# mcmilk/7-Zip-zstd

Measured on AMD Instinct MI355X. Metric: compress MB/s + ratio-vs-ref, enwik9 zstd-L3 & Silesia flzma2-L5 (value = the zstd-L3 enwik9 leg; flzma2_l5_silesia = the other leg), higher is better.
Workload: dtype u8; 1 GPU; zstd level 3, enwik9 stand-in (text-zipf, 1000000000 B), 128 KiB blocks in independent 8 MiB match-finder frames; bytes_total=1000000000

## Files before the change

7-zip-zstd_amd/csrc/gc_lz_window.hip:

```cpp
#include "gc_mf.h"
#include "gc_lz_parse.h"
#ifdef HIPEMU
#include <stdio.h>
#include <stdlib.h>
#endif

#ifdef GC_MF_FAST
#define MFK(name) name##_p8
#else
#define MFK(name) name
#endif

namespace MFK(gc_mf_ns) {

#define MF_T         GC_MF_PARTS
static_assert(MF_T == GC_MF_PARTS, "W1 uses one thread per partition for the histogram row");
#define MF_PWAVES    (GC_MF_PARTS / 64u)
#define MFS_T        GC_MF_SCATTER_T
#define MFS_WAVES    (MFS_T / 64u)
#define MFS_ROUNDS   (GC_MF_TILE / MFS_T)
static_assert(MFS_T >= GC_MF_PARTS && MFS_T % 64u == 0u && GC_MF_TILE % (2u * MFS_T) == 0u && GC_MF_PARTS < 0xFFFFu, "W3: the first GC_MF_PARTS threads do the offsets; whole rounds, two per register");
#define MF_STAGE_PAD 16u
#define MF_STAGE_WORDS ((GC_MF_TILE + 2u * MF_STAGE_PAD + 32u) / 4u)

// ... 226 lines not shown
    }
    __syncthreads();
    GcMfEntry* E = ent + (uint64_t)T.frame * ((uint64_t)MF_F(frameBlocks) * GC_ZSTD_BLOCK_MAX);
    for (uint32_t j = t; j < nEnt; j += MFS_T) {
        const MfKeys k = mf_keys<MODE>(sW, sPerm[j], T);
        E[sDelta[k.part] + j] = k.entry;
    }
}
extern "C" __global__ void __launch_bounds__(MFS_T)
MFK(gc_mf_scatter_kernel)(const uint8_t* __restrict__ src, uint64_t srcSize, uint32_t frameBlocks, uint32_t nTiles, uint32_t per,
                     const uint32_t* __restrict__ offs, GcMfEntry* __restrict__ ent)
{
    mf_scatter_body<MF_BASE>(src, srcSize, frameBlocks, nTiles, per, offs, ent);
}
extern "C" __global__ void __launch_bounds__(MFS_T)
MFK(gc_mf_scatter_short_kernel)(const uint8_t* __restrict__ src, uint64_t srcSize, uint32_t frameBlocks, uint32_t nTiles, uint32_t per,
                           const uint32_t* __restrict__ offs, GcMfEntry* __restrict__ ent)
{
    mf_scatter_body<MF_SHORT>(src, srcSize, frameBlocks, nTiles, per, offs, ent);
}
extern "C" __global__ void __launch_bounds__(MFS_T)
MFK(gc_mf_scatter_far_kernel)(const uint8_t* __restrict__ src, uint64_t srcSize, uint32_t frameBlocks, uint32_t nTiles, uint32_t per,
                         const uint32_t* __restrict__ offs, GcMfEntry* __restrict__ ent)
{
    mf_scatter_body<MF_FAR>(src, srcSize, frameBlocks, nTiles, per, offs, ent);
}
extern "C" __global__ void __launch_bounds__(MFS_T)
MFK(gc_mf_scatter_far2_kernel)(const uint8_t* __restrict__ src, uint64_t srcSize, uint32_t frameBlocks, uint32_t nTiles, uint32_t per,
                         const uint32_t* __restrict__ offs, GcMfEntry* __restrict__ ent)
{
    mf_scatter_body<MF_FAR2>(src, srcSize, frameBlocks, nTiles, per, offs, ent);
}

#ifndef LINK_DEPTH
#define LINK_DEPTH 8u
#endif
#ifdef GC_MF_FAST
#define LINK_SEG   49152u
#else
#define LINK_SEG   16384u
#endif
#define LINK_WARM  16384u
#define LINK_SEGS  GC_MF_LINK_SEGS
#define LINK_BATCH 16u

__device__ __forceinline__ uint32_t mf_link_pick(uint32_t seen, uint32_t mine)
{
    return (seen != 0u && seen < mine && ((seen ^ mine) & ((1u << GC_MF_TAG_BITS) - 1u)) == 0u) ? (seen >> GC_MF_TAG_BITS) : 0u;
}

__device__ __forceinline__ void mf_link_load(uint64_t q[LINK_DEPTH], const GcMfEntry* __restrict__ E, uint32_t s0, uint32_t end, uint32_t lane)
{
#pragma unroll
    for (uint32_t d = 0; d < LINK_DEPTH; d++) {
        const uint32_t i = s0 + d * 64u + lane;
        q[d] = E[i < end ? i : end - 1u];
    }
}

__device__ __forceinline__ void mf_link_steps(const uint64_t q[LINK_DEPTH], uint32_t* tabL, uint32_t* tabS, GcMfEntry* __restrict__ EO, uint32_t s0,
                                              uint32_t end, uint32_t lane)
{
    if (s0 >= end) return;
    uint32_t pos[LINK_DEPTH], mL[LINK_DEPTH], mS[LINK_DEPTH], rL[LINK_DEPTH], rS[LINK_DEPTH];
#pragma unroll
    for (uint32_t d = 0; d < LINK_DEPTH; d++) {
        const uint32_t i = s0 + d * 64u + lane;
        const uint64_t e = q[d];
        pos[d] = (uint32_t)e & ((1u << GC_MF_POS_BITS) - 1u);
        const uint32_t kL = (uint32_t)(e >> GC_MF_POS_BITS) & ((1u << GC_MF_KL_BITS) - 1u);
        const uint32_t kS = (uint32_t)(e >> (GC_MF_POS_BITS + GC_MF_KL_BITS)) & ((1u << GC_MF_KS_BITS) - 1u);
        mL[d] = ((pos[d] + 1u) << GC_MF_TAG_BITS) | (kL & ((1u << GC_MF_TAG_BITS) - 1u)); mS[d] = ((pos[d] + 1u) << GC_MF_TAG_BITS) | (kS & ((1u << GC_MF_TAG_BITS) - 1u));
        rL[d] = 0; rS[d] = 0;
        if (i < end) { rL[d] = atomicMax(&tabL[kL >> (GC_MF_KL_BITS - GC_MF_LSLOT_LOG)], mL[d]); rS[d] = atomicMax(&tabS[kS >> (GC_MF_KS_BITS - GC_MF_SSLOT_LOG)], mS[d]); }
        gc_wave_step();
    }
#pragma unroll
    for (uint32_t d = 0; d < LINK_DEPTH; d++) {
        const uint32_t i = s0 + d * 64u + lane;
        const uint32_t cL = mf_link_pick(rL[d], mL[d]), cS = mf_link_pick(rS[d], mS[d]);
        if (i < end) EO[i] = (uint64_t)(pos[d] & (GC_MF_TILE - 1u)) | ((uint64_t)cL << GC_MF_TILE_LOG) | ((uint64_t)cS << (GC_MF_TILE_LOG + GC_MF_CAND_BITS));
    }
}

extern "C" __global__ void __launch_bounds__(64)
MFK(gc_mf_link_kernel)(const uint32_t* __restrict__ offs, const GcMfEntry* __restrict__ ent, GcMfEntry* __restrict__ entOut, uint32_t tilesPerFrame,
                  uint64_t frameBytes, uint32_t nLists, uint32_t* __restrict__ ticket)
{
    __shared__ uint32_t tabL[1u << GC_MF_LSLOT_LOG];
    __shared__ uint32_t tabS[1u << GC_MF_SSLOT_LOG];
    const uint32_t lane = threadIdx.x;
    const uint32_t nUpper = nLists * (LINK_SEGS - 1u), nBatches = (nUpper + LINK_BATCH - 1u) / LINK_BATCH, nTickets = nBatches + nLists;
    for (;;) {
        uint32_t tk = 0;
        if (lane == 0u) tk = atomicAdd(ticket, 1u);
        tk = __shfl(tk, 0);
        if (tk >= nTickets) break;
        uint64_t todo;
        uint32_t myItem, myStart = 0, myEnd = 0;
        {
            myItem = tk < nBatches ? tk * LINK_BATCH + lane : nUpper + (tk - nBatches);
            const bool inRange = tk < nBatches ? (lane < LINK_BATCH && myItem < nUpper) : lane == 0u;
            bool exists = false;
            if (inRange) {
                const uint32_t seg = LINK_SEGS - 1u - myItem / nLists, fg = myItem % nLists;
                const uint32_t frame = fg >> GC_MF_PART_LOG, g = fg & (GC_MF_PARTS - 1u);
                const uint32_t* row = offs + (uint64_t)frame * (tilesPerFrame + 1u) * GC_MF_PARTS;
                const uint32_t listStart = row[g], listEnd = row[(uint64_t)tilesPerFrame * GC_MF_PARTS + g];
                myStart = listStart + seg * LINK_SEG;
                exists = myStart < listEnd;
                myEnd = (seg + 1u < LINK_SEGS && myStart + LINK_SEG < listEnd) ? myStart + LINK_SEG : listEnd;
            }
            todo = __ballot(exists);
        }
      while (todo != 0ull) {
        const uint32_t src_ = gc_ctz64(todo);
        todo &= todo - 1ull;
        const uint32_t item = __shfl(myItem, (int)src_), start = __shfl(myStart, (int)src_), end = __shfl(myEnd, (int)src_);
        const uint32_t seg = LINK_SEGS - 1u - item / nLists, fg = item % nLists;
        const uint32_t frame = fg >> GC_MF_PART_LOG;
        const GcMfEntry* E = ent + (uint64_t)frame * frameBytes;
        GcMfEntry* EO = entOut + (uint64_t)frame * frameBytes;
        gc_wave_sync();
        for (uint32_t i = lane; i < (1u << GC_MF_LSLOT_LOG); i += 64u) tabL[i] = 0;
        for (uint32_t i = lane; i < (1u << GC_MF_SSLOT_LOG); i += 64u) tabS[i] = 0;
        gc_wave_sync();
        if (seg != 0u) {
            for (uint32_t i = start - LINK_WARM + lane; i < start; i += 64u) {
                const uint64_t e = E[i];
                const uint32_t pos = (uint32_t)e & ((1u << GC_MF_POS_BITS) - 1u);
                const uint32_t kL = (uint32_t)(e >> GC_MF_POS_BITS) & ((1u << GC_MF_KL_BITS) - 1u);
                const uint32_t kS = (uint32_t)(e >> (GC_MF_POS_BITS + GC_MF_KL_BITS)) & ((1u << GC_MF_KS_BITS) - 1u);
                atomicMax(&tabL[kL >> (GC_MF_KL_BITS - GC_MF_LSLOT_LOG)], ((pos + 1u) << GC_MF_TAG_BITS) | (kL & ((1u << GC_MF_TAG_BITS) - 1u)));
                atomicMax(&tabS[kS >> (GC_MF_KS_BITS - GC_MF_SSLOT_LOG)], ((pos + 1u) << GC_MF_TAG_BITS) | (kS & ((1u << GC_MF_TAG_BITS) - 1u)));
            }
            gc_wave_sync();
        }
        uint64_t qa[LINK_DEPTH], qb[LINK_DEPTH];
        mf_link_load(qa, E, start, end, lane);
        for (uint32_t s0 = start; s0 < end; s0 += 2u * 64u * LINK_DEPTH) {
            mf_link_load(qb, E, s0 + 64u * LINK_DEPTH, end, lane);
            mf_link_steps(qa, tabL, tabS, EO, s0, end, lane);
            mf_link_load(qa, E, s0 + 2u * 64u * LINK_DEPTH, end, lane);
            mf_link_steps(qb, tabL, tabS, EO, s0 + 64u * LINK_DEPTH, end, lane);
        }
      }
    }
}

#define MFV_T GC_MF_VERIFY_T
#ifndef MFV_B
#define MFV_B 4u
#endif
#define MFV_NONE 0xFFFFFFFFu
#define MFV_PAD_AFTER (GC_MATCH_CAP + 32u)
#define MFV_STAGE_WORDS ((MF_STAGE_PAD + GC_MF_TILE + MFV_PAD_AFTER) / 4u)

__device__ __forceinline__ LzW16 mf_lds_ld16(const uint32_t* sW, uint32_t i)
{
    LzW16 w; w.a = mf_lds_ld64(sW, i); w.b = mf_lds_ld64(sW, i + 8u); return w;
}
__device__ __forceinline__ uint32_t mfv_len16(const LzW16& me, const LzW16& cw, uint32_t maxLen, uint32_t minLen = GC_MIN_MATCH)
{
    uint32_t len = lz_cmp16(me, cw);
    if (len > maxLen) len = maxLen;
    return len >= minLen ? len : 0u;
}

#define MFV_BACK 3u
__device__ __forceinline__ uint32_t mfv_len13(const LzW16& me, const LzW16& cw, uint32_t maxLen, uint32_t& ext, uint32_t minLen = GC_MIN_MATCH)
{
    const uint64_t d0 = me.a ^ cw.a, d1 = me.b ^ cw.b;
    const bool b2 = ((d0 >> 16) & 0xFFull) == 0ull, b1 = ((d0 >> 8) & 0xFFull) == 0ull, b0 = (d0 & 0xFFull) == 0ull;
    ext = b2 ? (b1 ? (b0 ? 3u : 2u) : 1u) : 0u;
    const uint64_t e0 = (d0 >> 24) | (d1 << 40), e1 = (d1 >> 24) | (1ull << 40);
    uint32_t len = e0 ? gc_ctz64(e0) >> 3 : 8u + (gc_ctz64(e1) >> 3);
    if (len > maxLen) len = maxLen;
    return len >= minLen ? len : 0u;
}

#define VP_PHASE(prof, tprev, i) do { if ((prof) != nullptr && threadIdx.x == 0) { const unsigned long long now_ = gc_clock(); atomicAdd(&(prof)[i], now_ - (tprev)); (tprev) = now_; } } while (0)

#define MFV_CATCH 3u
#define MFV_XBITS 0x80u
template <int MODE, bool TILE_LIMIT = false, bool BACK = false>
__device__ __forceinline__ void mf_verify_tile(const MfTile& T, const uint8_t* __restrict__ src, uint64_t srcSize, uint32_t frameBlocks,
                    const uint32_t* __restrict__ offs, const GcMfEntry* __restrict__ ent, const uint32_t* recIn,
                    uint32_t* sW, uint32_t* sRec, uint8_t* sExt, uint32_t* sStart, uint32_t* sLocal, uint32_t* sWaveTot,
                    unsigned long long* prof = nullptr, unsigned long long* tprev = nullptr,
                    const uint32_t* __restrict__ changedIn = nullptr )
{
    constexpr bool FAR = MODE == MF_FAR || MODE == MF_FAR2 || MODE == MF_SHORT;
    constexpr bool SHIFT = BACK;
    constexpr uint32_t MINLEN = MODE == MF_SHORT ? 3u : GC_MIN_MATCH;
    constexpr uint32_t LONGLEN = MODE == MF_SHORT ? 4u : ((MODE == MF_FAR || MODE == MF_FAR2) ? 16u : 8u);
    const uint32_t t = threadIdx.x, lane = t & 63u, wave = t >> 6;
    const uint32_t TPF = MF_F(frameBlocks) * GC_MF_TILES_PER_BLOCK;
    uint32_t c = 0, incl = 0;
    if (t < GC_MF_PARTS) {
        const uint32_t* row = offs + ((uint64_t)T.frame * (TPF + 1u) + T.tif) * GC_MF_PARTS;
        const uint32_t o = row[t];
        c = row[GC_MF_PARTS + t] - o;
        sStart[t] = o;
        incl = gc_wave_incl_sum(c);
        if (lane == 63u) sWaveTot[wave] = incl;
    }
    mf_stage(sW, MFV_STAGE_WORDS, src, srcSize, T.tileStart, t, MFV_T);
    uint32_t* const sDirty = (uint32_t*)sExt;
    uint32_t* const sBack2 = (uint32_t*)(sExt + GC_MF_TILE / 8u + 16u);
    if (BACK) { for (uint32_t i = t; i < GC_MF_TILE / 32u; i += MFV_T) sBack2[i] = 0u; }
    if (FAR) {
        const GcU4* R4 = (const GcU4*)(recIn + T.tileStart);
        GcU4* S4 = (GcU4*)sRec;
        for (uint32_t i = t; i < (T.len + 3u) / 4u; i += MFV_T) S4[i] = R4[i];
        const uint32_t* D = changedIn != nullptr ? changedIn + (T.tileStart >> 5) : (const uint32_t*)nullptr;
        const uint32_t nW = (T.len + 31u) / 32u;
        for (uint32_t i = t; i < GC_MF_TILE / 32u + 4u; i += MFV_T) sDirty[i] = D != nullptr ? ((i < nW ? D[i] : 0u) | ((i >= 2u && i - 2u < nW) ? D[i - 2u] : 0u)) : 0u;
    } else {
        GcU4 none; none.x = none.y = none.z = none.w = MFV_NONE;
        GcU4* S4 = (GcU4*)sRec;
        for (uint32_t i = t; i < GC_MF_TILE / 4u; i += MFV_T) S4[i] = none;
    }
    __syncthreads();
    if (t < GC_MF_PARTS) {
        uint32_t before = 0;
        for (uint32_t w = 0; w < GC_MF_PARTS / 64u; w++) if (w < wave) before += sWaveTot[w];
        sLocal[t] = before + incl - c;
        if (t == GC_MF_PARTS - 1u) sLocal[GC_MF_PARTS] = before + incl;
    }
    __syncthreads();
    const uint32_t nEnt = sLocal[GC_MF_PARTS];
    VP_PHASE(prof, *tprev, 0);
    const uint8_t* wsrc = src + T.frameStart;
    const GcMfEntry* E = ent + (uint64_t)T.frame * ((uint64_t)MF_F(frameBlocks) * GC_ZSTD_BLOCK_MAX);
    const uint64_t blockBase = T.tileStart & ~(uint64_t)(GC_ZSTD_BLOCK_MAX - 1u);
    const uint32_t nBlk = (uint32_t)((srcSize - blockBase) < GC_ZSTD_BLOCK_MAX ? (srcSize - blockBase) : GC_ZSTD_BLOCK_MAX);
    const uint32_t pTile = (uint32_t)(T.tileStart - blockBase);
    const uint32_t wTile = (uint32_t)(T.tileStart - T.frameStart);
    auto unlisted = [&]() {
        for (uint32_t q = t; q < T.len; q += MFV_T) {
            if (!FAR && sRec[q] != MFV_NONE) continue;
            const uint64_t x = mf_lds_ld64(sW, q + MF_STAGE_PAD);
            const bool run = T.tileStart + q > T.frameStart && ((x << 8) | (uint64_t)mf_lds_byte(sW, q + MF_STAGE_PAD - 1u)) == x;
            const bool windowed = T.tileStart + q + GC_MATCH_CAP + 16u <= T.frameEnd;
            if (windowed && !run) continue;
            const uint32_t p = pTile + q;
            uint32_t len = 0;
            if (run && windowed && p + 8u <= nBlk) {
                uint32_t maxLen = (nBlk - p) < GC_MATCH_CAP ? (nBlk - p) : GC_MATCH_CAP;
                if (TILE_LIMIT && maxLen > T.len - q) maxLen = T.len - q;
                while (len < maxLen) {
                    const uint32_t more = lz_cmp16(mf_lds_ld16(sW, q + MF_STAGE_PAD + len), mf_lds_ld16(sW, q + MF_STAGE_PAD - 1u + len));
                    len += more;
                    if (more < 16u) break;
                }
                if (len > maxLen) len = maxLen;
                if (len < GC_MIN_MATCH) len = 0;
            }
            sRec[q] = len ? ((1u << 8) | len) : 0u;
        }
    };
    const uint32_t stagedLo = wTile >= MF_STAGE_PAD ? wTile - MF_STAGE_PAD : wTile + 0xFFFFFFFFu , stagedHi = wTile + (MFV_STAGE_WORDS * 4u - MF_STAGE_PAD);
    auto ld16c = [&](uint64_t c) -> LzW16 {
        if (wTile >= MF_STAGE_PAD && c >= stagedLo && c + 20u <= stagedHi) return mf_lds_ld16(sW, (uint32_t)(c - stagedLo));
        return lz_ld16(wsrc, c);
    };
    const uint32_t perWave = ((nEnt + MFV_T - 1u) / MFV_T) * 64u;
    const uint32_t jBeg = wave * perWave, jEnd = jBeg + perWave < nEnt ? jBeg + perWave : nEnt;
    uint32_t g0 = 0;
    if (jBeg < jEnd) {
#pragma unroll
        for (uint32_t step = GC_MF_PARTS / 2u; step != 0u; step >>= 1) if (sLocal[g0 + step] <= jBeg) g0 += step;
    }
    for (uint32_t j0 = jBeg; j0 < jEnd; j0 += 64u * MFV_B) {
        uint64_t e[MFV_B];
        bool live[MFV_B];
#pragma unroll
        for (uint32_t k = 0; k < MFV_B; k++) {
            const uint32_t j = j0 + k * 64u + lane;
            live[k] = j < jEnd;
            const uint32_t jj = live[k] ? j : jEnd - 1u;
            uint32_t lo = g0;
            while (sLocal[lo + 1u] <= jj) lo++;
            e[k] = E[sStart[lo] + (jj - sLocal[lo])];
            g0 = gc_readlane(lo, 63u);
        }
        uint32_t q[MFV_B], cS[MFV_B], maxLen[MFV_B], bestLen[MFV_B], bestC[MFV_B];
        uint32_t bestExt[MFV_B];
        LzW16 cw[MFV_B];
#pragma unroll
        for (uint32_t k = 0; k < MFV_B; k++) {
            q[k] = (uint32_t)e[k] & (GC_MF_TILE - 1u);
            const uint32_t cL = (uint32_t)(e[k] >> GC_MF_TILE_LOG) & ((1u << GC_MF_CAND_BITS) - 1u);
            cS[k] = (uint32_t)(e[k] >> (GC_MF_TILE_LOG + GC_MF_CAND_BITS)) & ((1u << GC_MF_CAND_BITS) - 1u);
            const uint32_t p = pTile + q[k];
            const bool can = live[k] && p + 8u <= nBlk;
            maxLen[k] = can ? ((nBlk - p) < GC_MATCH_CAP ? (nBlk - p) : GC_MATCH_CAP) : 0u;
            if (TILE_LIMIT && maxLen[k] > T.len - q[k]) maxLen[k] = T.len - q[k];
            if (cS[k] == cL) cS[k] = 0;
            bestC[k] = (can && cL) ? cL : 0u;
            bestExt[k] = 0;
            if (SHIFT) { if (bestC[k] <= MFV_BACK) bestC[k] = 0; if (cS[k] <= MFV_BACK) cS[k] = 0; }
            if (bestC[k]) cw[k] = ld16c(bestC[k] - 1u - (SHIFT ? MFV_BACK : 0u));
        }
#pragma unroll
        for (uint32_t k = 0; k < MFV_B; k++) {
            if (SHIFT) { uint32_t x = 0; bestLen[k] = bestC[k] ? mfv_len13(mf_lds_ld16(sW, q[k] + MF_STAGE_PAD - MFV_BACK), cw[k], maxLen[k], x, MINLEN) : 0u; bestExt[k] = (BACK && x > q[k]) ? q[k] : x; }
            else bestLen[k] = bestC[k] ? mfv_len16(mf_lds_ld16(sW, q[k] + MF_STAGE_PAD), cw[k], maxLen[k], MINLEN) : 0u;
            if (bestLen[k] >= (SHIFT && LONGLEN > 13u ? 13u : LONGLEN) || maxLen[k] == 0u) cS[k] = 0;
            if (cS[k]) cw[k] = ld16c(cS[k] - 1u - (SHIFT ? MFV_BACK : 0u));
        }
#pragma unroll
        for (uint32_t k = 0; k < MFV_B; k++) {
            const uint32_t pw = wTile + q[k];
            if (cS[k]) {
                uint32_t x = 0;
                const uint32_t len = SHIFT ? mfv_len13(mf_lds_ld16(sW, q[k] + MF_STAGE_PAD - MFV_BACK), cw[k], maxLen[k], x, MINLEN) : mfv_len16(mf_lds_ld16(sW, q[k] + MF_STAGE_PAD), cw[k], maxLen[k], MINLEN);
                if (BACK && x > q[k]) x = q[k];
                if (len && (bestLen[k] == 0u || lz_gain(len, pw - (cS[k] - 1u)) > lz_gain(bestLen[k], pw - (bestC[k] - 1u)))) { bestLen[k] = len; bestC[k] = cS[k]; bestExt[k] = x; }
            }
            uint32_t len = bestLen[k];
            while ((SHIFT ? (len & 15u) == 13u : (len >= 16u && (len & 15u) == 0u)) && len < maxLen[k]) {
                const uint32_t more = lz_cmp16(mf_lds_ld16(sW, q[k] + MF_STAGE_PAD + len), ld16c((uint64_t)(bestC[k] - 1u) + len));
                len += more;
                if (len > maxLen[k]) len = maxLen[k];
                if (more < 16u) break;
            }
            if (live[k]) {
                const uint32_t nr = len ? (((pw - (bestC[k] - 1u)) << 8) | len) : 0u;
                if (MODE == MF_BASE && len == GC_MATCH_CAP) sWaveTot[1] = 0xFFFFFFFFu;
                const uint32_t xb = (BACK && nr != 0u) ? ((bestExt[k] & 1u) << 7) : 0u;
                const bool x2 = BACK && nr != 0u && (bestExt[k] & 2u) != 0u;
                if (!FAR) { sRec[q[k]] = nr | xb; if (x2) atomicOr(&sBack2[q[k] >> 5], 1u << (q[k] & 31u)); }
                else if (nr) {
                    const uint32_t old = sRec[q[k]];
                    bool take = old == 0u || lz_gain(len, nr >> 8) > lz_gain(old & 0xFFu, old >> 8);
                    if (MODE == MF_FAR2 && old != 0u && len == GC_MATCH_CAP && (old & 0xFFu) == GC_MATCH_CAP && (old >> 8) != (nr >> 8)) {
                        const uint64_t frameLen = T.frameEnd - T.frameStart;
                        const uint64_t room = frameLen - ((uint64_t)pw + GC_MATCH_CAP);
                        const uint32_t lim = room < 80u ? (room < 16u ? 0u : (uint32_t)room - 16u) : 64u;
                        uint32_t eN = 0, eO = 0;
                        const uint64_t own = (uint64_t)pw + GC_MATCH_CAP;
                        while (eN < lim) { const uint32_t m = lz_cmp16(lz_ld16(wsrc, own + eN), lz_ld16(wsrc, own - (nr >> 8) + eN)); eN += m; if (m < 16u) break; }
                        while (eO < lim) { const uint32_t m = lz_cmp16(lz_ld16(wsrc, own + eO), lz_ld16(wsrc, own - (old >> 8) + eO)); eO += m; if (m < 16u) break; }
                        if (eN > lim) eN = lim; if (eO > lim) eO = lim;
                        take = eN > eO || (eN == eO && (nr >> 8) < (old >> 8));
                    }
                    if (take) {
                        sRec[q[k]] = nr | xb; if (x2) atomicOr(&sBack2[q[k] >> 5], 1u << (q[k] & 31u));
                        atomicOr(&sDirty[q[k] >> 5], 1u << (q[k] & 31u)); atomicOr(&sDirty[(q[k] + GC_MATCH_CAP) >> 5], 1u << ((q[k] + GC_MATCH_CAP) & 31u));
                    }
                }
            }
        }
    }
    VP_PHASE(prof, *tprev, 1);
    if (!FAR) { __syncthreads(); unlisted(); }
    if (BACK) {
        __syncthreads();
        constexpr uint32_t NSUBC = MFV_T / 64u;
        const uint32_t shareLen = GC_MF_TILE / NSUBC, cBeg = wave * shareLen, cEnd = cBeg + shareLen;
        uint32_t beyond[MFV_CATCH];
#pragma unroll
        for (uint32_t j = 0; j < MFV_CATCH; j++) beyond[j] = cEnd + j < T.len ? sRec[cEnd + j] : 0u;
        __syncthreads();
        for (uint32_t x0 = cBeg; x0 < cEnd && x0 < T.len; x0 += 64u) {
            const uint32_t x = x0 + lane;
            const uint32_t old = x < T.len ? sRec[x] : 0u;
            const uint32_t own = old & ~MFV_XBITS;
            uint32_t best = own;
            int bg = (own & 0xFFu) ? lz_gain(own & 0xFFu, own >> 8) : -100000;
#pragma unroll
            for (uint32_t j = 1; j <= MFV_CATCH; j++) {
                const uint32_t y = x + j;
                uint32_t ry = (y < cEnd && y < T.len) ? sRec[y] : 0u;
                if (y >= cEnd) ry = y - cEnd == 0u ? beyond[0] : (y - cEnd == 1u ? beyond[1] : beyond[2]);
                const uint32_t e = (ry & 0x7Fu) == 0u ? 0u : (((ry >> 7) & 1u) | (((sBack2[(y & (GC_MF_TILE - 1u)) >> 5] >> (y & 31u)) & 1u) << 1));
                if (e >= j) {
                    uint32_t l = (ry & 0x7Fu) + j; if (l > GC_MATCH_CAP) l = GC_MATCH_CAP;
                    const uint32_t off = ry >> 8;
                    const int g = lz_gain(l, off);
                    if (g > bg) { bg = g; best = (off << 8) | l; }
                }
            }
            gc_wave_sync();
            if (x < T.len && old != best) {
                sRec[x] = best;
                if (own != best) {
                    if (FAR) { atomicOr(&sDirty[x >> 5], 1u << (x & 31u)); atomicOr(&sDirty[(x + GC_MATCH_CAP) >> 5], 1u << ((x + GC_MATCH_CAP) & 31u)); }
                    if (MODE == MF_BASE && (best & 0xFFu) == GC_MATCH_CAP) sWaveTot[1] = 0xFFFFFFFFu;
                }
            }
            gc_wave_sync();
        }
    }
    __syncthreads();
    if ((MODE == MF_BASE && sWaveTot[1] == 0xFFFFFFFFu) || MODE == MF_FAR || MODE == MF_FAR2 || MODE == MF_SHORT) {
        constexpr uint32_t NSUB = MFV_T / 64u;
        const uint32_t subLen = ((T.len + NSUB * 64u - 1u) / (NSUB * 64u)) * 64u;
        const uint32_t sBeg = wave * subLen, sEnd = sBeg + subLen < T.len ? sBeg + subLen : T.len;
        auto piece4 = [&](uint32_t q, uint64_t cpos, uint32_t maxLen, const LzW16& c0, const LzW16& c1, const LzW16& c2, const LzW16& c3) -> uint32_t {
            const bool h1 = 16u < maxLen, h2 = 32u < maxLen, h3 = 48u < maxLen;
            uint32_t more = lz_cmp16(mf_lds_ld16(sW, q + MF_STAGE_PAD), c0);
            bool full = more == 16u;
            if (full && h1) { const uint32_t m = lz_cmp16(mf_lds_ld16(sW, q + MF_STAGE_PAD + 16u), c1); more += m; full = m == 16u; }
            if (full && h2) { const uint32_t m = lz_cmp16(mf_lds_ld16(sW, q + MF_STAGE_PAD + 32u), c2); more += m; full = m == 16u; }
            if (full && h3) { const uint32_t m = lz_cmp16(mf_lds_ld16(sW, q + MF_STAGE_PAD + 48u), c3); more += m; full = m == 16u; }
            (void)cpos;
            return more > maxLen ? maxLen : more;
        };
        auto walk = [&](uint32_t q, const uint32_t qEnd, const bool follow) {
            while (q < qEnd) {
                const uint32_t prev = sRec[q - GC_MATCH_CAP];
                const uint32_t d = prev >> 8, cur = sRec[q];
                const uint32_t p = pTile + q;
                const bool fresh = !FAR || ((sDirty[q >> 5] >> (q & 31u)) & 1u) != 0u;
                const bool need0 = fresh && (prev & 0xFFu) == GC_MATCH_CAP && (cur >> 8) != d && d <= wTile + q
                                   && T.tileStart + q + GC_MATCH_CAP + 16u <= T.frameEnd && p + 8u <= nBlk;
                if (!need0) { if (follow) return; q += 64u; continue; }
                uint32_t max0 = (nBlk - p) < GC_MATCH_CAP ? (nBlk - p) : GC_MATCH_CAP;
                if (TILE_LIMIT && max0 > T.len - q) max0 = T.len - q;
                const uint64_t cpos = (uint64_t)(wTile + q) - d;
                const uint32_t q1 = q + 64u;
                uint32_t cur1 = 0u;
                bool spec = max0 == GC_MATCH_CAP && q1 < qEnd;
                if (spec) {
                    cur1 = sRec[q1];
                    spec = (cur1 >> 8) != d && T.tileStart + q1 + GC_MATCH_CAP + 16u <= T.frameEnd && p + 64u + GC_MATCH_CAP <= nBlk && (!TILE_LIMIT || q1 + GC_MATCH_CAP <= T.len);
                }
                const bool h1 = 16u < max0, h2 = 32u < max0, h3 = 48u < max0;
                const LzW16 c0 = lz_ld16(wsrc, cpos), c1 = lz_ld16(wsrc, cpos + (h1 ? 16u : 0u)), c2 = lz_ld16(wsrc, cpos + (h2 ? 32u : 0u)), c3 = lz_ld16(wsrc, cpos + (h3 ? 48u : 0u));
                LzW16 e0 = c0, e1 = c0, e2 = c0, e3 = c0;
                if (spec) { e0 = lz_ld16(wsrc, cpos + 64u); e1 = lz_ld16(wsrc, cpos + 80u); e2 = lz_ld16(wsrc, cpos + 96u); e3 = lz_ld16(wsrc, cpos + 112u); }
                const uint32_t len0 = piece4(q, cpos, max0, c0, c1, c2, c3);
                if (len0 < MINLEN || len0 + 2u < (cur & 0xFFu)) { if (follow) return; q += 64u; continue; }
                sRec[q] = (d << 8) | len0;
                if (FAR) atomicOr(&sDirty[q1 >> 5], 1u << (q1 & 31u));
                if (!(spec && len0 == GC_MATCH_CAP)) { q += 64u; continue; }
                const uint32_t len1 = piece4(q1, cpos + 64u, GC_MATCH_CAP, e0, e1, e2, e3);
                if (len1 < MINLEN || len1 + 2u < (cur1 & 0xFFu)) { if (follow) return; q += 128u; continue; }
                sRec[q1] = (d << 8) | len1;
                if (FAR) atomicOr(&sDirty[(q1 + 64u) >> 5], 1u << ((q1 + 64u) & 31u));
                q += 128u;
            }
        };
        walk(sBeg + GC_MATCH_CAP + lane, sEnd, false);
        __syncthreads();
        const uint32_t qFirst = sBeg + lane;
        const uint32_t prevA = (wave != 0u && qFirst < sEnd) ? sRec[qFirst - GC_MATCH_CAP] : 0u;
        __syncthreads();
        if (wave != 0u) walk(qFirst, sEnd, true);
        __syncthreads();
        for (uint32_t sIdx = 2; sIdx < NSUB; sIdx++) {
            if (wave == sIdx && qFirst < sEnd && sRec[qFirst - GC_MATCH_CAP] != prevA) walk(qFirst, sEnd, true);
            __syncthreads();
        }
    }
}

template <int MODE, bool BACK = true>
__device__ __forceinline__ void mf_verify_body(const uint8_t* __restrict__ src, uint64_t srcSize, uint32_t frameBlocks, uint32_t nTiles, uint32_t per,
                    const uint32_t* __restrict__ offs, const GcMfEntry* __restrict__ ent, const uint32_t* recIn, uint32_t* rec, const uint32_t* __restrict__ changedIn = nullptr)
{
    __shared__ uint32_t sW[MFV_STAGE_WORDS];
    __shared__ uint32_t sRec[GC_MF_TILE];
    __shared__ __attribute__((aligned(16))) uint8_t sExt[2u * (GC_MF_TILE / 8u + 16u)];
    __shared__ uint32_t sStart[GC_MF_PARTS], sLocal[GC_MF_PARTS + 1u];
    __shared__ uint32_t sWaveTot[GC_MF_PARTS / 64u];
    const uint32_t t = threadIdx.x;
    const uint32_t tile = mf_item(blockIdx.x, per);
    if (tile >= nTiles) return;
    const MfTile T = mf_tile(tile, frameBlocks, srcSize);
    if (T.len == 0u || !T.own) return;
    mf_verify_tile<MODE, false, BACK>(T, src, srcSize, frameBlocks, offs, ent, recIn, sW, sRec, sExt, sStart, sLocal, sWaveTot, nullptr, nullptr, changedIn);
    GcU4* R4 = (GcU4*)(rec + T.tileStart);
    const GcU4* S4 = (const GcU4*)sRec;
    for (uint32_t i = t; i < (T.len + 3u) / 4u; i += MFV_T) R4[i] = S4[i];
}
extern "C" __global__ void __launch_bounds__(MFV_T)
MFK(gc_mf_verify_kernel)(const uint8_t* __restrict__ src, uint64_t srcSize, uint32_t frameBlocks, uint32_t nTiles, uint32_t per,
                    const uint32_t* __restrict__ offs, const GcMfEntry* __restrict__ ent, uint32_t* __restrict__ rec)
{
    mf_verify_body<MF_BASE>(src, srcSize, frameBlocks, nTiles, per, offs, ent, rec, rec);
}
extern "C" __global__ void __launch_bounds__(MFV_T)
MFK(gc_mf_verify_far_kernel)(const uint8_t* __restrict__ src, uint64_t srcSize, uint32_t frameBlocks, uint32_t nTiles, uint32_t per,
                        const uint32_t* __restrict__ offs, const GcMfEntry* __restrict__ ent, uint32_t* __restrict__ rec)
{
    mf_verify_body<MF_FAR>(src, srcSize, frameBlocks, nTiles, per, offs, ent, rec, rec);
}
extern "C" __global__ void __launch_bounds__(MFV_T)
MFK(gc_mf_verify_far2_kernel)(const uint8_t* __restrict__ src, uint64_t srcSize, uint32_t frameBlocks, uint32_t nTiles, uint32_t per,
                        const uint32_t* __restrict__ offs, const GcMfEntry* __restrict__ ent, uint32_t* __restrict__ rec)
{
    mf_verify_body<MF_FAR2>(src, srcSize, frameBlocks, nTiles, per, offs, ent, rec, rec);
}
extern "C" __global__ void __launch_bounds__(MFV_T)
MFK(gc_mf_verify_short_kernel)(const uint8_t* __restrict__ src, uint64_t srcSize, uint32_t frameBlocks, uint32_t nTiles, uint32_t per,
                          const uint32_t* __restrict__ offs, const GcMfEntry* __restrict__ ent, const uint32_t* __restrict__ recIn, uint32_t* __restrict__ recOut,
                          const uint32_t* __restrict__ changedIn)
{
    mf_verify_body<MF_SHORT, false>(src, srcSize, frameBlocks, nTiles, per, offs, ent, recIn, recOut, changedIn);
}
extern "C" __global__ void __launch_bounds__(MFV_T)
MFK(gc_mf_verify_shortb_kernel)(const uint8_t* __restrict__ src, uint64_t srcSize, uint32_t frameBlocks, uint32_t nTiles, uint32_t per,
                          const uint32_t* __restrict__ offs, const GcMfEntry* __restrict__ ent, const uint32_t* __restrict__ recIn, uint32_t* __restrict__ recOut,
                          const uint32_t* __restrict__ changedIn)
{
    mf_verify_body<MF_SHORT, true>(src, srcSize, frameBlocks, nTiles, per, offs, ent, recIn, recOut, changedIn);
}

#define MFD_T 256u
#define MFD_LONG 32u
extern "C" __global__ void __launch_bounds__(MFD_T)
MFK(gc_mf_deepen_kernel)(const uint8_t* __restrict__ src, uint64_t srcSize, uint32_t frameBlocks, uint32_t nTiles, uint32_t per, uint32_t depths ,
                    const uint32_t* __restrict__ recIn, uint32_t* __restrict__ recOut,
                    uint32_t* __restrict__ changed )
{
    __shared__ uint32_t sLong;
    const uint32_t depth = depths & 0xFFu, shallow = depths >> 8;
    const uint32_t t = threadIdx.x;
    const uint32_t tile = mf_item(blockIdx.x, per);
    if (tile >= nTiles) return;
    const MfTile T = mf_tile(tile, frameBlocks, srcSize);
    if (T.len == 0u || !T.own) return;
    const uint8_t* wsrc = src + T.frameStart;
    const uint32_t* RI = recIn + T.frameStart;
    const uint64_t blockBase = T.tileStart & ~(uint64_t)(GC_ZSTD_BLOCK_MAX - 1u);
    const uint32_t nBlk = (uint32_t)((srcSize - blockBase) < GC_ZSTD_BLOCK_MAX ? (srcSize - blockBase) : GC_ZSTD_BLOCK_MAX);
    const uint32_t pTile = (uint32_t)(T.tileStart - blockBase), wTile = (uint32_t)(T.tileStart - T.frameStart);
    if (t == 0u) sLong = 0;
    __syncthreads();
    uint32_t nLong = 0;
    for (uint32_t q = t; q < T.len; q += MFD_T) nLong += (RI[wTile + q] & 0xFFu) >= MFD_LONG ? 1u : 0u;
    nLong = gc_wave_sum(nLong);
    if ((t & 63u) == 0u && nLong) atomicAdd(&sLong, nLong);
    __syncthreads();
    const uint32_t depthStart = sLong * 16u >= T.len ? depth : shallow;
    for (uint32_t q0 = 0; q0 < T.len; q0 += MFD_T) {
        const uint32_t q = q0 + t;
        const bool in = q < T.len;
        const uint32_t pw = wTile + q, p = pTile + q;
        const uint32_t r = in ? RI[pw] : 0u;
        uint32_t bestLen = r & 0xFFu, bestOff = r >> 8;
        if (bestLen != 0u && bestLen < GC_MATCH_CAP && T.tileStart + q + GC_MATCH_CAP + 16u <= T.frameEnd) {
            const uint32_t rp = pw ? RI[pw - 1u] : 0u;
            const bool inside = (rp >> 8) == bestOff && (rp & 0xFFu) > bestLen;
            const uint32_t nLinks = inside ? shallow : depthStart;
            const uint32_t maxLen = (nBlk - p) < GC_MATCH_CAP ? (nBlk - p) : GC_MATCH_CAP;
            const LzW16 me = lz_ld16(wsrc, pw);
            int bestGain = lz_gain(bestLen, bestOff);
            uint32_t c = pw - bestOff;
            for (uint32_t d = 0; d < nLinks; d++) {
                const uint32_t rc = RI[c];
                if ((rc & 0xFFu) == 0u || (rc >> 8) > c) break;
                const uint32_t c2 = c - (rc >> 8);
                uint32_t len = lz_cmp16(me, lz_ld16(wsrc, c2));
                while (len >= 16u && (len & 15u) == 0u && len < maxLen) {
                    const uint32_t more = lz_cmp16(lz_ld16(wsrc, (uint64_t)pw + len), lz_ld16(wsrc, (uint64_t)c2 + len));
                    len += more;
                    if (more < 16u) break;
                }
                if (len > maxLen) len = maxLen;
                if (len >= GC_MIN_MATCH) { const int g = lz_gain(len, pw - c2); if (g > bestGain) { bestGain = g; bestLen = len; bestOff = pw - c2; } }
                c = c2;
            }
        }
        const uint32_t nr = (bestOff << 8) | bestLen;
        if (in) recOut[T.tileStart + q] = nr;
        if (changed != nullptr) {
            const uint64_t m = __ballot(in && nr != r);
            if ((t & 63u) == 0u && q < ((T.len + 63u) & ~63u)) { uint32_t* W = changed + ((T.tileStart + q) >> 5); W[0] = (uint32_t)m; W[1] = (uint32_t)(m >> 32); }
        }
    }
}

#define PZ_T       GC_MF_PARSE_T
#define PZ_WAVES   (PZ_T / 64u)
#define PZ_GSEGS   32u
#define PZ_GROUPS  (GC_ZSTD_BLOCK_MAX / 64u / PZ_GSEGS)

struct PzSeg { uint32_t r0; bool take; uint32_t nxt; };
__device__ __forceinline__ PzSeg pz_seg(const uint32_t* __restrict__ R, uint32_t p, uint32_t n, uint32_t lane, uint32_t lazy)
{
    PzSeg s;
    s.r0 = p < n ? R[p] : 0u;
    const uint32_t r1 = p + 1u < n ? R[p + 1u] : 0u;
    const uint32_t len = s.r0 & 0xFFu, l1 = r1 & 0xFFu;
    s.take = len != 0u;
    const int g0 = lz_gain(len, s.r0 >> 8);
    if (lazy >= 1u && s.take && l1 > len && lz_gain(l1, r1 >> 8) > g0 + 4) s.take = false;
    if (lazy >= 2u) {
        const uint32_t r2 = p + 2u < n ? R[p + 2u] : 0u;
        const uint32_t l2 = r2 & 0xFFu;
        if (s.take && l2 > len + 1u && lz_gain(l2, r2 >> 8) > g0 + 8) s.take = false;
    }
    s.nxt = s.take ? lane + len : lane + 1u;
    return s;
}
__device__ __forceinline__ uint32_t pz_exit(uint32_t nxt)
{
    uint32_t cur = nxt;
#pragma unroll
    for (int r = 0; r < 6; r++) { const uint32_t o = __shfl(cur, (int)(cur & 63u)); if (cur < 64u) cur = o; }
    return cur;
}


#define VP_WAVES   (MFV_T / 64u)
#define VP_SEGS    (GC_MF_TILE / 64u)
#define VP_SPW     (VP_SEGS / VP_WAVES)
#if defined(GC_MF_FAST)
#define VP_MIN_WAVES 6
#else
#define VP_MIN_WAVES 4
#endif
extern "C" __global__ void __launch_bounds__(MFV_T, VP_MIN_WAVES)
MFK(gc_mf_vparse_tile_kernel)(const uint8_t* __restrict__ src, uint64_t srcSize, uint32_t frameBlocks, uint32_t nTiles, uint32_t per ,
                    uint32_t lazy, const uint32_t* __restrict__ offs, const GcMfEntry* __restrict__ ent,
                    GcSeqRaw* __restrict__ seqRaw, uint8_t* __restrict__ lit, GcBlockMeta* __restrict__ meta,
                    uint32_t* __restrict__ tickets , uint32_t* __restrict__ tileWord ,
                    unsigned long long* __restrict__ prof)
{
    __shared__ uint32_t sW[MFV_STAGE_WORDS];
    __shared__ uint32_t sRec[GC_MF_TILE];
    __shared__ uint8_t sExt[4u];
    __shared__ uint32_t sAux[GC_MF_TILE / 4u];
    static_assert(VP_SPW % 4u == 0u && VP_SPW <= 64u, "the parse keeps a wave's exit maps four to a register and walks one segment per lane");
    uint32_t* sStart = sAux; uint32_t* sLocal = sAux + GC_MF_PARTS; uint32_t* sWaveTot = sAux + 2u * GC_MF_PARTS + 1u;
    uint8_t* sNxt = (uint8_t*)sAux;
    __shared__ uint8_t  sExitW[VP_WAVES][64];
    __shared__ uint64_t sMaskSeq[VP_SEGS], sMaskLit[VP_SEGS];
    __shared__ uint32_t sCntSeq[VP_WAVES], sCntLit[VP_WAVES];
    __shared__ uint32_t sTicket, sBase[2];
    const uint32_t t = threadIdx.x, lane = t & 63u, wave = t >> 6;
    if (t == 0) sTicket = atomicAdd(&tickets[blockIdx.x & (GC_XCDS - 1u)], 1u);
    __syncthreads();
    const uint32_t tile = (blockIdx.x & (GC_XCDS - 1u)) * per + sTicket;
    if (tile >= nTiles) return;
    const MfTile T = mf_tile(tile, frameBlocks, srcSize);
    if (T.len == 0u) return;
    unsigned long long tprev = prof ? gc_clock() : 0ull;
    const uint32_t b = tile / GC_MF_TILES_PER_BLOCK, ti = tile % GC_MF_TILES_PER_BLOCK;
    GcSeqRaw* mySeq = seqRaw + (uint64_t)b * GC_MAX_SEQ_PER_BLOCK;
    uint8_t* myLit = lit + (uint64_t)b * GC_ZSTD_BLOCK_MAX;
    const uint64_t lt = gc_lanemask_lt();
    mf_verify_tile<MF_BASE, true>(T, src, srcSize, frameBlocks, offs, ent, nullptr, sW, sRec, sExt, sStart, sLocal, sWaveTot, prof, &tprev);
    const uint32_t n = T.len;
    VP_PHASE(prof, tprev, 2);
    const uint32_t seg0 = wave * VP_SPW;
    uint32_t x4[VP_SPW / 4u];
    {
        uint32_t comp = lane;
#pragma unroll
        for (uint32_t g = 0; g < VP_SPW / 4u; g++) {
            uint32_t m[4];
#pragma unroll
            for (uint32_t j = 0; j < 4u; j++) {
                const uint32_t k = 4u * g + j, seg = seg0 + k;
                const PzSeg s = pz_seg(sRec, seg * 64u + lane, n, lane, lazy);
                sNxt[seg * 64u + lane] = (uint8_t)s.nxt;
                m[j] = pz_exit(s.nxt) - 64u;
                const uint64_t tk = __ballot(s.take);
                if (lane == 0) sMaskSeq[seg] = tk;
            }
            x4[g] = m[0] | (m[1] << 8) | (m[2] << 16) | (m[3] << 24);
            m[0] = __shfl(m[1], (int)m[0]); m[2] = __shfl(m[3], (int)m[2]); m[0] = __shfl(m[2], (int)m[0]);
            comp = __shfl(m[0], (int)comp);
            gc_sched_fence();
        }
        sExitW[wave][lane] = (uint8_t)comp;
    }
    __syncthreads();
    VP_PHASE(prof, tprev, 3);
    uint32_t e = 0;
    for (uint32_t w = 0; w < wave; w++) e = sExitW[w][e];
    e = gc_uniform(e);
    uint32_t myE = 0;
#pragma unroll
    for (uint32_t k = 0; k < VP_SPW; k++) {
        myE = gc_writelane(myE, e, k);
        e = (gc_readlane(x4[k >> 2], e) >> (8u * (k & 3u))) & 0xFFu;
    }
    uint32_t cnt = 0;
    {
        const uint32_t seg = seg0 + lane;
        const bool mine = lane < VP_SPW && seg * 64u < n;
        const uint32_t lim = mine ? (n - seg * 64u < 64u ? n - seg * 64u : 64u) : 0u;
        const uint8_t* row = sNxt + (mine ? seg * 64u : 0u);
        uint64_t path = 0;
        uint32_t c = myE;
        for (uint32_t i = 0; i < 64u && c < lim; i++) { path |= 1ull << c; c = row[c]; }
        if (mine) {
            const uint64_t myTake = sMaskSeq[seg];
            const uint64_t mS = path & myTake, mL = path & ~myTake;
            sMaskSeq[seg] = mS; sMaskLit[seg] = mL;
            cnt = ((uint32_t)__popcll(mS) << 16) | (uint32_t)__popcll(mL);
        }
    }
    cnt = gc_wave_sum(cnt);
    if (lane == 0) { sCntSeq[wave] = cnt >> 16; sCntLit[wave] = cnt & 0xFFFFu; }
    __syncthreads();
    VP_PHASE(prof, tprev, 4);
    uint32_t sBefore = 0, lBefore = 0, sAll = 0, lAll = 0;
    for (uint32_t w = 0; w < VP_WAVES; w++) {
        const uint32_t cs = sCntSeq[w], cl = sCntLit[w];
        if (w < wave) { sBefore += cs; lBefore += cl; }
        sAll += cs; lAll += cl;
    }
    if (wave == 0) {
        if (lane == 0) {
#ifdef HIPEMU
            __atomic_store_n(&tileWord[tile], 0x80000000u | (sAll << 15) | lAll, __ATOMIC_RELEASE);
#else
            __hip_atomic_store(&tileWord[tile], 0x80000000u | (sAll << 15) | lAll, __ATOMIC_RELAXED, __HIP_MEMORY_SCOPE_AGENT);
#endif
        }
        uint32_t w = 0x80000000u;
        if (lane < ti) { uint32_t spins = 0; do { w = gc_poll_device(&tileWord[tile - ti + lane]); if (!(w >> 31)) { gc_nap(); if (++spins > (1u << 22)) { atomicOr(tickets - 1, 1u); w = 0x80000000u; } } } while (!(w >> 31)); }
        const uint32_t sb = gc_wave_sum(lane < ti ? (w >> 15) & 0xFFFFu : 0u), lb = gc_wave_sum(lane < ti ? w & 0x7FFFu : 0u);
        if (lane == 0) { sBase[0] = sb; sBase[1] = lb; }
    }
    __syncthreads();
    VP_PHASE(prof, tprev, 5);
    const uint32_t seqBase = sBase[0], litBase = sBase[1];
    uint32_t sr = seqBase + sBefore, lr = litBase + lBefore;
#pragma unroll 1
    for (uint32_t k = 0; k < VP_SPW; k++) {
        const uint32_t seg = seg0 + k;
        if (seg * 64u >= n) break;
        const uint64_t mS = sMaskSeq[seg], mL = sMaskLit[seg];
        const uint32_t q = seg * 64u + lane;
        const uint32_t myLitRank = lr + (uint32_t)__popcll(mL & lt);
        if ((mS >> lane) & 1ull) { GcSeqRaw r; r.litRank = myLitRank; r.offml = sRec[q]; mySeq[sr + (uint32_t)__popcll(mS & lt)] = r; }
        if ((mL >> lane) & 1ull) myLit[myLitRank] = (uint8_t)mf_lds_byte(sW, q + MF_STAGE_PAD);
        sr += (uint32_t)__popcll(mS); lr += (uint32_t)__popcll(mL);
    }
    const bool lastOfBlock = ti + 1u == GC_MF_TILES_PER_BLOCK || T.tileStart + n >= T.frameEnd;
    if (t == 0 && lastOfBlock) { GcBlockMeta m; m.nSeqRaw = seqBase + sAll; m.nLit = litBase + lAll; meta[b] = m; }
    VP_PHASE(prof, tprev, 6);
}

#ifndef GC_MF_FAST
#define PZR_G0   4
#define PZR_GK   1
#define PZR_LAZY 7
#define PZR_LPS 16u
#define PZR_MAX_STREAMS 16u
__device__ __forceinline__ uint32_t pzr_eq16(LzW16 x, LzW16 y)
{
    uint32_t m = 0;
    const uint32_t d[4] = { (uint32_t)(x.a ^ y.a), (uint32_t)((x.a ^ y.a) >> 32), (uint32_t)(x.b ^ y.b), (uint32_t)((x.b ^ y.b) >> 32) };
#pragma unroll
    for (uint32_t i = 0; i < 4u; i++) {
        const uint32_t nzb = (((d[i] & 0x7F7F7F7Fu) + 0x7F7F7F7Fu) | d[i]) & 0x80808080u;
        const uint32_t eq = (~nzb & 0x80808080u) >> 7;
        m |= (((eq * 0x00204081u) >> 21) & 0xFu) << (4u * i);
    }
    return m;
}
extern "C" __global__ void __launch_bounds__(256)
gc_mf_ringparse_kernel(const uint8_t* __restrict__ src, uint64_t srcSize, uint32_t nBlocks, uint32_t per, uint32_t lazy, uint32_t ringMin, const uint32_t* __restrict__ rec,
                       GcSeqRaw* __restrict__ seqRaw, uint8_t* __restrict__ lit, GcBlockMeta* __restrict__ meta)
{
    __shared__ uint32_t sCntS[PZR_MAX_STREAMS], sCntL[PZR_MAX_STREAMS];
    const uint32_t t = threadIdx.x, lane = t & 63u, T = blockDim.x, nStreams = T / PZR_LPS;
    const uint32_t b = mf_item(blockIdx.x, per);
    if (b >= nBlocks) return;
    const uint64_t base = (uint64_t)b * GC_ZSTD_BLOCK_MAX;
    const uint32_t n = (uint32_t)((srcSize - base) < GC_ZSTD_BLOCK_MAX ? (srcSize - base) : GC_ZSTD_BLOCK_MAX);
    const uint32_t* R = rec + base;
    GcSeqRaw* mySeq = seqRaw + (uint64_t)b * GC_MAX_SEQ_PER_BLOCK;
    uint8_t* myLit = lit + (uint64_t)b * GC_ZSTD_BLOCK_MAX;
    const uint8_t* bsrc = src + base;
    const uint32_t st = t / PZR_LPS, j = t % PZR_LPS, k = j >> 2, ch = j & 3u, g0 = lane & ~(PZR_LPS - 1u);
    const uint32_t sub = ((n + nStreams * 64u - 1u) / (nStreams * 64u)) * 64u;
    const uint32_t seqCap = GC_MAX_SEQ_PER_BLOCK / nStreams;
    const uint32_t p0 = st * sub, pEnd = p0 < n ? (n - p0 < sub ? n : p0 + sub) : p0;
    const uint32_t ringLim = (srcSize - base) >= 96u ? (uint32_t)((srcSize - base - 96u) < n ? (srcSize - base - 96u) : n) : 0u;
    GcSeqRaw* sq = mySeq + st * seqCap;
    uint8_t* lq = myLit + p0;
    const uint32_t quietMin = (ringMin >> 16) & 0xFFu, warm = (ringMin >> 24) * 16u, selShift = (ringMin >> 8) & 0xFFu;
    ringMin &= 0xFFu;
    if (selShift) {
        __shared__ uint32_t sSel;
        if (t == 0u) sSel = 0u;
        __syncthreads();
        const uint32_t nRaw = meta[b].nSeqRaw, nScan = nRaw < 4096u ? nRaw : 4096u;
        uint32_t cnt = 0;
        for (uint32_t i = 3u + t; i < nScan; i += T) {
            const GcSeqRaw a = mySeq[i], a1 = mySeq[i - 1u], a2 = mySeq[i - 2u], a3 = mySeq[i - 3u];
            const uint32_t o = a.offml >> 8, o1 = a1.offml >> 8;
            if (o == o1 ? a.litRank != a1.litRank : (o == (a2.offml >> 8) || o == (a3.offml >> 8))) cnt++;
        }
        cnt = gc_wave_sum(cnt);
        if (lane == 0u && cnt) atomicAdd(&sSel, cnt);
        __shared__ uint32_t sGo, sSeen;
        if (t == 0u) { sGo = 0u; sSeen = 0u; }
        __syncthreads();
        uint32_t go = 0, seen = 0;
// ... 248 lines not shown
```

Before: 49220 MB/s.

## Defer saturated match extension in base verify to a compacted work queue

In the non-far verify modes, saturated matches are no longer extended inline inside the per-thread candidate loop. Their positions are pushed into a shared-memory queue with wave ballots and atomics. The queue is drained in full-block batches during the unlisted pass, which is meant to remove divergence from long serial extension loops. In exchange it adds extra __syncthreads barriers, an atomic counter and queue storage in LDS that shares space with sAux in vparse.

```diff
diff --git a/7-zip-zstd_amd/csrc/gc_lz_window.hip b/7-zip-zstd_amd/csrc/gc_lz_window.hip
--- a/7-zip-zstd_amd/csrc/gc_lz_window.hip
+++ b/7-zip-zstd_amd/csrc/gc_lz_window.hip
@@ -402,6 +402,12 @@
 #ifndef MFV_B
 #define MFV_B 4u
 #endif
+#if defined(GC_MF_FAST)
+#define MFV_QG 4u
+#else
+#define MFV_QG 2u
+#endif
+#define MFV_QCAP ((MFV_QG + 1u) * MFV_T)
 #define MFV_NONE 0xFFFFFFFFu
 #define MFV_PAD_AFTER (GC_MATCH_CAP + 32u)
 #define MFV_STAGE_WORDS ((MF_STAGE_PAD + GC_MF_TILE + MFV_PAD_AFTER) / 4u)
@@ -437,6 +443,7 @@
 __device__ __forceinline__ void mf_verify_tile(const MfTile& T, const uint8_t* __restrict__ src, uint64_t srcSize, uint32_t frameBlocks,
                     const uint32_t* __restrict__ offs, const GcMfEntry* __restrict__ ent, const uint32_t* recIn,
                     uint32_t* sW, uint32_t* sRec, uint8_t* sExt, uint32_t* sStart, uint32_t* sLocal, uint32_t* sWaveTot,
+                    uint16_t* sQ , uint32_t* sQn,
                     unsigned long long* prof = nullptr, unsigned long long* tprev = nullptr,
                     const uint32_t* __restrict__ changedIn = nullptr )
 {
@@ -470,6 +477,7 @@
         GcU4 none; none.x = none.y = none.z = none.w = MFV_NONE;
         GcU4* S4 = (GcU4*)sRec;
         for (uint32_t i = t; i < GC_MF_TILE / 4u; i += MFV_T) S4[i] = none;
+        if (t == 0u) *sQn = 0u;
     }
     __syncthreads();
     if (t < GC_MF_PARTS) {
@@ -487,33 +495,84 @@
     const uint32_t nBlk = (uint32_t)((srcSize - blockBase) < GC_ZSTD_BLOCK_MAX ? (srcSize - blockBase) : GC_ZSTD_BLOCK_MAX);
     const uint32_t pTile = (uint32_t)(T.tileStart - blockBase);
     const uint32_t wTile = (uint32_t)(T.tileStart - T.frameStart);
-    auto unlisted = [&]() {
-        for (uint32_t q = t; q < T.len; q += MFV_T) {
-            if (!FAR && sRec[q] != MFV_NONE) continue;
-            const uint64_t x = mf_lds_ld64(sW, q + MF_STAGE_PAD);
-            const bool run = T.tileStart + q > T.frameStart && ((x << 8) | (uint64_t)mf_lds_byte(sW, q + MF_STAGE_PAD - 1u)) == x;
-            const bool windowed = T.tileStart + q + GC_MATCH_CAP + 16u <= T.frameEnd;
-            if (windowed && !run) continue;
-            const uint32_t p = pTile + q;
-            uint32_t len = 0;
-            if (run && windowed && p + 8u <= nBlk) {
-                uint32_t maxLen = (nBlk - p) < GC_MATCH_CAP ? (nBlk - p) : GC_MATCH_CAP;
-                if (TILE_LIMIT && maxLen > T.len - q) maxLen = T.len - q;
-                while (len < maxLen) {
-                    const uint32_t more = lz_cmp16(mf_lds_ld16(sW, q + MF_STAGE_PAD + len), mf_lds_ld16(sW, q + MF_STAGE_PAD - 1u + len));
-                    len += more;
-                    if (more < 16u) break;
-                }
-                if (len > maxLen) len = maxLen;
-                if (len < GC_MIN_MATCH) len = 0;
-            }
-            sRec[q] = len ? ((1u << 8) | len) : 0u;
-        }
-    };
     const uint32_t stagedLo = wTile >= MF_STAGE_PAD ? wTile - MF_STAGE_PAD : wTile + 0xFFFFFFFFu , stagedHi = wTile + (MFV_STAGE_WORDS * 4u - MF_STAGE_PAD);
     auto ld16c = [&](uint64_t c) -> LzW16 {
         if (wTile >= MF_STAGE_PAD && c >= stagedLo && c + 20u <= stagedHi) return mf_lds_ld16(sW, (uint32_t)(c - stagedLo));
         return lz_ld16(wsrc, c);
+    };
+    auto saturated = [&](uint32_t len) -> bool { return SHIFT ? (len & 15u) == 13u : (len >= 16u && (len & 15u) == 0u); };
+    auto extend = [&](uint32_t n) {
+        for (uint32_t i = t; i < n; i += MFV_T) {
+            const uint32_t q = sQ[i], rec = sRec[q];
+            const uint32_t p = pTile + q;
+            uint32_t maxLen = (nBlk - p) < GC_MATCH_CAP ? (nBlk - p) : GC_MATCH_CAP;
+            if (TILE_LIMIT && maxLen > T.len - q) maxLen = T.len - q;
+            const uint64_t c = (uint64_t)(wTile + q) - (rec >> 8);
+            uint32_t len = rec & 0x7Fu;
+            while (len < maxLen) {
+                const uint32_t more = lz_cmp16(mf_lds_ld16(sW, q + MF_STAGE_PAD + len), ld16c(c + len));
+                len += more;
+                if (len > maxLen) len = maxLen;
+                if (more < 16u) break;
+            }
+            sRec[q] = (rec & ~0x7Fu) | len;
+            if (MODE == MF_BASE && len == GC_MATCH_CAP) sWaveTot[1] = 0xFFFFFFFFu;
+        }
+    };
+    auto unlisted = [&]() {
+        uint32_t step = 0;
+        for (uint32_t q0 = 0; q0 < T.len; q0 += MFV_T) {
+            const uint32_t q = q0 + t;
+            bool sat = false;
+            const uint32_t rec = q < T.len ? sRec[q] : 0u;
+            if (q < T.len && rec != MFV_NONE) {
+                if (saturated(rec & 0x7Fu)) {
+                    const uint32_t p = pTile + q;
+                    uint32_t maxLen = p + 8u <= nBlk ? ((nBlk - p) < GC_MATCH_CAP ? (nBlk - p) : GC_MATCH_CAP) : 0u;
+                    if (TILE_LIMIT && maxLen > T.len - q) maxLen = T.len - q;
+                    sat = (rec & 0x7Fu) < maxLen;
+                }
+            } else if (q < T.len) {
+                const uint64_t x = mf_lds_ld64(sW, q + MF_STAGE_PAD);
+                const bool run = T.tileStart + q > T.frameStart && ((x << 8) | (uint64_t)mf_lds_byte(sW, q + MF_STAGE_PAD - 1u)) == x;
+                const bool windowed = T.tileStart + q + GC_MATCH_CAP + 16u <= T.frameEnd;
+                if (!windowed || run) {
+                    const uint32_t p = pTile + q;
+                    uint32_t len = 0;
+                    if (run && windowed && p + 8u <= nBlk) {
+                        uint32_t maxLen = (nBlk - p) < GC_MATCH_CAP ? (nBlk - p) : GC_MATCH_CAP;
+                        if (TILE_LIMIT && maxLen > T.len - q) maxLen = T.len - q;
+                        while (len < maxLen) {
+                            const uint32_t more = lz_cmp16(mf_lds_ld16(sW, q + MF_STAGE_PAD + len), mf_lds_ld16(sW, q + MF_STAGE_PAD - 1u + len));
+                            len += more;
+                            if (more < 16u) break;
+                        }
+                        if (len > maxLen) len = maxLen;
+                        if (len < GC_MIN_MATCH) len = 0;
+                    }
+                    sRec[q] = len ? ((1u << 8) | len) : 0u;
+                }
+            }
+            const uint64_t m = __ballot(sat);
+            if (m != 0ull) {
+                uint32_t at = 0;
+                if (lane == 0u) at = atomicAdd(sQn, (uint32_t)__popcll(m));
+                at = gc_readlane(at, 0u);
+                if (sat) sQ[at + (uint32_t)__popcll(m & gc_lanemask_lt())] = (uint16_t)q;
+            }
+            const bool last = q0 + MFV_T >= T.len;
+            if (++step == MFV_QG || last) {
+                step = 0;
+                __syncthreads();
+                const uint32_t n = *sQn;
+                __syncthreads();
+                if (n >= MFV_T || (last && n != 0u)) {
+                    if (t == 0u) *sQn = 0u;
+                    extend(n);
+                    __syncthreads();
+                }
+            }
+        }
     };
     const uint32_t perWave = ((nEnt + MFV_T - 1u) / MFV_T) * 64u;
     const uint32_t jBeg = wave * perWave, jEnd = jBeg + perWave < nEnt ? jBeg + perWave : nEnt;
@@ -570,7 +629,7 @@
                 if (len && (bestLen[k] == 0u || lz_gain(len, pw - (cS[k] - 1u)) > lz_gain(bestLen[k], pw - (bestC[k] - 1u)))) { bestLen[k] = len; bestC[k] = cS[k]; bestExt[k] = x; }
             }
             uint32_t len = bestLen[k];
-            while ((SHIFT ? (len & 15u) == 13u : (len >= 16u && (len & 15u) == 0u)) && len < maxLen[k]) {
+            while (FAR && saturated(len) && len < maxLen[k]) {
                 const uint32_t more = lz_cmp16(mf_lds_ld16(sW, q[k] + MF_STAGE_PAD + len), ld16c((uint64_t)(bestC[k] - 1u) + len));
                 len += more;
                 if (len > maxLen[k]) len = maxLen[k];
@@ -604,8 +663,8 @@
             }
         }
     }
+    if (!FAR) { __syncthreads(); unlisted(); }
     VP_PHASE(prof, *tprev, 1);
-    if (!FAR) { __syncthreads(); unlisted(); }
     if (BACK) {
         __syncthreads();
         constexpr uint32_t NSUBC = MFV_T / 64u;
@@ -717,12 +776,17 @@
     __shared__ __attribute__((aligned(16))) uint8_t sExt[2u * (GC_MF_TILE / 8u + 16u)];
     __shared__ uint32_t sStart[GC_MF_PARTS], sLocal[GC_MF_PARTS + 1u];
     __shared__ uint32_t sWaveTot[GC_MF_PARTS / 64u];
+    constexpr bool FIRST = MODE == MF_BASE;
+    __shared__ uint16_t sQ[FIRST ? MFV_QCAP : 2u];
+    __shared__ uint32_t sQn;
+    static_assert(sizeof(sW) + sizeof(sRec) + sizeof(sExt) + sizeof(sStart) + sizeof(sLocal) + sizeof(sWaveTot) + sizeof(uint16_t) * MFV_QCAP + sizeof(sQn) + 8u * 64u
+                  <= (160u * 1024u) / (MFV_T == 512u ? 3u : 1u), "the stand-alone verify no longer fits its workgroups per CU");
     const uint32_t t = threadIdx.x;
     const uint32_t tile = mf_item(blockIdx.x, per);
     if (tile >= nTiles) return;
     const MfTile T = mf_tile(tile, frameBlocks, srcSize);
     if (T.len == 0u || !T.own) return;
-    mf_verify_tile<MODE, false, BACK>(T, src, srcSize, frameBlocks, offs, ent, recIn, sW, sRec, sExt, sStart, sLocal, sWaveTot, nullptr, nullptr, changedIn);
+    mf_verify_tile<MODE, false, BACK>(T, src, srcSize, frameBlocks, offs, ent, recIn, sW, sRec, sExt, sStart, sLocal, sWaveTot, sQ, &sQn, nullptr, nullptr, changedIn);
     GcU4* R4 = (GcU4*)(rec + T.tileStart);
     const GcU4* S4 = (const GcU4*)sRec;
     for (uint32_t i = t; i < (T.len + 3u) / 4u; i += MFV_T) R4[i] = S4[i];
@@ -878,6 +942,8 @@
     __shared__ uint32_t sAux[GC_MF_TILE / 4u];
     static_assert(VP_SPW % 4u == 0u && VP_SPW <= 64u, "the parse keeps a wave's exit maps four to a register and walks one segment per lane");
     uint32_t* sStart = sAux; uint32_t* sLocal = sAux + GC_MF_PARTS; uint32_t* sWaveTot = sAux + 2u * GC_MF_PARTS + 1u;
+    uint32_t* sQn = sWaveTot + GC_MF_PARTS / 64u; uint16_t* sQ = (uint16_t*)(sQn + 1u);
+    static_assert(2u * GC_MF_PARTS + 1u + GC_MF_PARTS / 64u + 1u + MFV_QCAP / 2u <= GC_MF_TILE / 4u, "the run table and the queue share sAux");
     uint8_t* sNxt = (uint8_t*)sAux;
     __shared__ uint8_t  sExitW[VP_WAVES][64];
     __shared__ uint64_t sMaskSeq[VP_SEGS], sMaskLit[VP_SEGS];
@@ -895,7 +961,7 @@
     GcSeqRaw* mySeq = seqRaw + (uint64_t)b * GC_MAX_SEQ_PER_BLOCK;
     uint8_t* myLit = lit + (uint64_t)b * GC_ZSTD_BLOCK_MAX;
     const uint64_t lt = gc_lanemask_lt();
-    mf_verify_tile<MF_BASE, true>(T, src, srcSize, frameBlocks, offs, ent, nullptr, sW, sRec, sExt, sStart, sLocal, sWaveTot, prof, &tprev);
+    mf_verify_tile<MF_BASE, true>(T, src, srcSize, frameBlocks, offs, ent, nullptr, sW, sRec, sExt, sStart, sLocal, sWaveTot, sQ, sQn, prof, &tprev);
     const uint32_t n = T.len;
     VP_PHASE(prof, tprev, 2);
     const uint32_t seg0 = wave * VP_SPW;
```

After: 49940 MB/s, median of 6. +1.5%, better.
